# ouguangjun/Leg-KILO

Measured on NVIDIA H100. Metric: LiDAR point-iterations/sec through the ESKF point-to-plane update, higher is better.
Workload: dtype f64

## Files before the change

leg-kilo_b200/csrc/lk_api.cu:

```cuda
#include <cmath>
#include <cstdio>
#include <chrono>
#include <cstring>
#include <mutex>
#include <string>
#include <vector>

#include "lk_host.h"
#include "lk_kernels.h"
#include "lk_mapdev.h"

namespace lk {
int decode_pointcloud2_device(const uint8_t* h_data, uint32_t n, const lk_pc2_layout& L, float blind, int filter_num,
                              double time_scale, float* h_pts_out, float* h_intensity_out, uint32_t* n_out, cudaStream_t s,
                              std::string& err);
int preprocess_scan_device(const float* h_pts_in, uint32_t n, float leaf, float* h_pts_out, uint32_t* n_out,
                           uint32_t* h_bucket_offsets, float* h_bucket_curv, uint32_t* n_buckets, cudaStream_t s,
                           std::string& err);
size_t leg_kinematics_scratch_bytes(uint32_t n);
int leg_kinematics_device(const lk_leg_cfg& cfg, const lk_leg_state* h_in, uint32_t n, int redundancy,
                          lk_leg_track* track, lk_kinimu_meas* h_out, uint32_t* n_out, void* scratch, cudaStream_t s,
                          std::string& err);
}

// ... 22 lines not shown
          Q(clk + align256((size_t)batch * sizeof(lk_stream_clock))),
          chunksL(Q + align256(900 * 8)),
          initsL(chunksL + align256(n_chunksL * sizeof(ChunkDesc))),
          bytes(initsL + align256(n_initsL * sizeof(StepInit))) {}
};

struct OutBlock {
    size_t x = 0, P = 0, clk = 0, n_eff = 0, status = 0, bytes = 0;
    OutBlock() = default;
    explicit OutBlock(int batch)
        : P(align256((size_t)batch * sizeof(lk_state))),
          clk(P + align256((size_t)batch * 900 * 8)),
          n_eff(clk + align256((size_t)batch * sizeof(lk_stream_clock))),
          status(n_eff + align256((size_t)batch * 4)),
          bytes(status + 256) {}
};

}

struct lk_context {
    int device = 0;
    cudaStream_t stream = nullptr;
    std::string err;
    lk_eskf_cfg ec;
    lk_map_cfg mc;
    Globals g;

    MapDevHost map;
    double last_slide_position[3] = {0.0, 0.0, 0.0};

    int batch = 0;
    uint64_t total_pts = 0;
    uint32_t total_chunks = 0, n_steps = 0, max_chunk_pts = 0;
    std::vector<ChunkDesc> h_chunks, h_chunksL;
    InBlock in;
    OutBlock out;
    DevBuf pts, world, sc, step, partial, ticket, fb_list, fb_cnt;
    DevBuf small_in, small_out, fx, fP, fQ, fclk;
    PinnedBuf h_small_in, h_small_out;
    DevView chunks, stepinit, x_in, P_in, clk_in, Q, x, P, clk, n_eff, status;
    DevBuf dbg_ok, dbg_h, dbg_z, dbg_R, dbg_key, tmp, trace, bar;
    DevBuf ins_pts, ins_root, ins_pend, ins_touched, ins_counters, ins_list;
    uint64_t ins_pend_nodes = 0;
    DevBuf mi_pts, mi_small, mi_ipts, mi_root, mi_touched, mi_counters, mi_list;
    PinnedBuf h_mi;
    int trace_on = 0;
    uint32_t trace_seq = 0;
    int lane_cache = 1;
    int use_fused = 1;
    FusedInline inl;
    DevBuf ll;
    uint32_t ll_epoch = 1;
    bool prev_fused = false;
    uint32_t fused_launches = 0, fused_launches_since_check = 0;
    int direct_io = 1, inline_in = 1, coop_launch = 0, pdl = 1, n_sms = 132, slim_p = 1;
    int finishers = 1;
    int fast_insert = 1;
    int fused_insert = 0;
    int debug_records = 0;
    bool direct = false, direct_ran = false, inline_ok = false;
    const float4* direct_pts = nullptr;
    float4* direct_world = nullptr;
    double hprof[8] = {0, 0, 0, 0, 0, 0, 0, 0};
    DevBuf Qc;
    DevBuf leg_scratch;
    std::vector<double> Q_shadow;

    cudaEvent_t ev0 = nullptr, ev1 = nullptr;
    std::vector<cudaEvent_t> kev;
    float last_total_ms = 0, last_residual_ms = 0;
    uint32_t last_launches = 0, last_residual_launches = 0;
    uint32_t acc_launches = 0, acc_residual_launches = 0;
    size_t nev = 0;
    int kernel_timing = 1;
    std::vector<StepInit> h_inits;
    std::vector<uint32_t> h_scan_pts;
    std::vector<uint32_t> h_scan_chunks;
    std::vector<StepInit> h_initsL;
    DevView chunksL, stepinitL;
    uint32_t total_chunksL = 0;

    ~lk_context() {
        for (cudaEvent_t e : kev) cudaEventDestroy(e);
        if (ev0) cudaEventDestroy(ev0);
        if (ev1) cudaEventDestroy(ev1);
        if (stream) cudaStreamDestroy(stream);
    }
};

namespace {

int fail(lk_handle h, int code, const std::string& msg) {
    if (h) h->err = msg;
    else g_create_error = msg;
    return code;
}

struct FusedGate {
    std::mutex m;
    cudaStream_t last = nullptr;
    cudaEvent_t ev = nullptr;
};
FusedGate& fused_gate(int device) {
    static FusedGate gates[64];
    return gates[(device >= 0 && device < 64) ? device : 0];
}

void enter(lk_handle h) {
    cudaSetDevice(h->device);
// ... 181 lines not shown
int lk_init_process_cov(const lk_eskf_cfg* c, double* Q) {
    if (!c || !Q) return LK_ERR_INVALID_ARG;
    for (int i = 0; i < 900; ++i) Q[i] = 0.0;
    const double d[7] = {c->vel_process_cov,     c->acc_bias_process_cov, c->gyr_bias_process_cov, c->imu_acc_process_cov,
                         c->imu_gyr_process_cov, c->kin_bias_process_cov, c->contact_process_cov};
    const int at[7] = {6, 9, 12, 18, 21, 24, 27};
    for (int b = 0; b < 7; ++b)
        for (int k = 0; k < 3; ++k) Q[(at[b] + k) * 30 + at[b] + k] = d[b];
    return LK_OK;
}

int lk_state_default(lk_state* x) {
    if (!x) return LK_ERR_INVALID_ARG;
    std::memset(x, 0, sizeof(*x));
    x->rot[0] = x->rot[4] = x->rot[8] = 1.0;
    x->grav[2] = -9.81;
    return LK_OK;
}

int lk_leg_track_default(lk_leg_track* t) {
    if (!t) return LK_ERR_INVALID_ARG;
    for (int k = 0; k < 4; ++k) t->in_contact[k] = 1;
    t->last_acc_z = 0.0f;
    t->last_gyr_z = 0.0f;
    return LK_OK;
}

int lk_host_alloc(void** p, size_t bytes) {
    if (!p) return LK_ERR_INVALID_ARG;
    cudaError_t e = cudaHostAlloc(p, bytes, cudaHostAllocDefault);
    if (e != cudaSuccess) {
        cudaGetLastError();
        return LK_ERR_OUT_OF_MEMORY;
    }
    return LK_OK;
}

int lk_host_free(void* p) {
    if (p) cudaFreeHost(p);
    return LK_OK;
}

int lk_set_param(lk_handle h, const char* name, double value) {
    if (!h || !name) return LK_ERR_INVALID_ARG;
    using IntKnob = int lk_context::*;
    static const struct {
        const char* name;
        IntKnob knob;
    } knobs[] = {{"kernel_timing", &lk_context::kernel_timing}, {"fused", &lk_context::use_fused},
                 {"lane_cache", &lk_context::lane_cache},       {"fast_insert", &lk_context::fast_insert},
                 {"fused_insert", &lk_context::fused_insert},   {"coop_launch", &lk_context::coop_launch},
                 {"pdl", &lk_context::pdl},                     {"slim_p", &lk_context::slim_p},
                 {"direct_io", &lk_context::direct_io},         {"inline_in", &lk_context::inline_in},
                 {"debug_records", &lk_context::debug_records}, {"finishers", &lk_context::finishers}};
    for (const auto& k : knobs)
        if (!std::strcmp(name, k.name)) {
            h->*k.knob = (int)value;
            return LK_OK;
        }
    if (!std::strcmp(name, "trace")) {
        h->trace_on = (int)value;
        if (h->trace_on) {
            enter(h);
            LK_CUDA(h->err, h->trace.ensure((size_t)(1 << 16) * 8 * 8));
            LK_CUDA(h->err, cudaMemset(h->trace.p, 0, (size_t)(1 << 16) * 8 * 8));
        }
        h->trace_seq = 0;
        return LK_OK;
    }
    return fail(h, LK_ERR_INVALID_ARG, std::string("unknown parameter ") + name);
}

int lk_debug_read(lk_handle h, int what, void* dst, size_t bytes) {
    if (!h || !dst) return LK_ERR_INVALID_ARG;
    if (what == 3) {
        std::memcpy(dst, h->hprof, std::min(bytes, sizeof(h->hprof)));
        std::memset(h->hprof, 0, sizeof(h->hprof));
        return LK_OK;
    }
    enter(h);
    DevBuf* b = what == 0 ? &h->partial : (what == 1 ? &h->sc : &h->trace);
    if (what == 2) h->trace_seq = 0;
    if (bytes > b->cap) bytes = b->cap;
    LK_CUDA(h->err, cudaMemcpy(dst, b->p, bytes, cudaMemcpyDeviceToHost));
    return LK_OK;
}

int lk_sync(lk_handle h) {
    if (!h) return LK_ERR_INVALID_ARG;
    enter(h);
    LK_CUDA(h->err, cudaStreamSynchronize(h->stream));
    return check_stall(h);
}


int lk_map_reserve(lk_handle h, uint64_t max_roots, uint64_t max_nodes, uint64_t max_points) {
    if (!h) return LK_ERR_INVALID_ARG;
    h->map.reserve_roots = max_roots;
    h->map.reserve_nodes = max_nodes;
    h->map.reserve_points = max_points;
    return LK_OK;
}

int lk_map_upload(lk_handle h, const void* blob, size_t bytes) {
    if (!h || !blob) return fail(h, LK_ERR_INVALID_ARG, "null argument");
    enter(h);
    return map_upload_blob(h->map, h->g, blob, bytes, h->stream, h->err);
// ... 158 lines not shown
                    cd.scan = (uint32_t)s;
                    cd.start = q;
                    cd.count = std::min(cs, p1 - q);
                    cd.pad = 0;
                    chunks.push_back(cd);
                }
                in.chunk_end = (uint32_t)chunks.size();
            }
        }
    };
    std::vector<ChunkDesc>& chunks = h->h_chunks;
    std::vector<ChunkDesc>& chunksL = h->h_chunksL;
    std::vector<StepInit>& inits = h->h_inits;
    build_tables(false, chunks, inits);
    bool twoTables = false;
    if (batch >= 2) {
        for (uint32_t b = 0; b < scan_bucket_ptr[batch] && !twoTables; ++b) {
            const uint32_t n = bucket_offsets[b + 1] - bucket_offsets[b];
            twoTables = chunk_size_for(n, true, big_chunk) != chunk_size_for(n, false);
        }
    }
    if (twoTables) build_tables(true, chunksL, h->h_initsL);
    else { chunksL.clear(); h->h_initsL.clear(); }
    h->batch = batch;
    h->h_scan_pts.assign(batch, 0);
    h->h_scan_chunks.assign(batch, 1);
    for (int s2 = 0; s2 < batch; ++s2) {
        h->h_scan_pts[s2] = scan_offsets[s2 + 1] - scan_offsets[s2];
        for (uint32_t k = 0; k < max_buckets; ++k) {
            const StepInit& in = inits[(size_t)k * batch + s2];
            h->h_scan_chunks[s2] = std::max(h->h_scan_chunks[s2], in.chunk_end - in.chunk_begin);
        }
    }
    h->total_pts = total;
    h->total_chunks = (uint32_t)chunks.size();
    h->max_chunk_pts = 0;
    for (const ChunkDesc& cd : chunks) h->max_chunk_pts = std::max(h->max_chunk_pts, cd.count);
    h->n_steps = max_buckets;

    LK_CUDA(h->err, h->pts.ensure(std::max<size_t>(total, 1) * 16));
    LK_CUDA(h->err, h->world.ensure(std::max<size_t>(total, 1) * 16));
    LK_CUDA(h->err, h->sc.ensure((size_t)batch * sizeof(ScanConst)));
    LK_CUDA(h->err, h->step.ensure((size_t)batch * sizeof(ScanStep)));
    LK_CUDA(h->err, h->partial.ensure(2 * std::max<size_t>(std::max(chunks.size(), chunksL.size()), 1) * PARTIAL_STRIDE * 8));
    if (batch >= 2 || h->max_chunk_pts > 256) {
        const size_t nch = std::max<size_t>(std::max(chunks.size(), chunksL.size()), 1);
        LK_CUDA(h->err, h->fb_list.ensure(nch * S2_FB_WARPS * S2_FB_CAP * sizeof(uint16_t)));
        LK_CUDA(h->err, h->fb_cnt.ensure(nch * S2_FB_WARPS * sizeof(uint32_t)));
    }
    if (!h->ll.p) {
        LK_CUDA(h->err, h->ll.ensure(LL_BYTES));
        LK_CUDA(h->err, cudaMemsetAsync(h->ll.p, 0, LL_BYTES, h->stream));
        h->ll_epoch = 1;
    }
    LK_CUDA(h->err, h->ticket.ensure((size_t)batch * 4));
    const InBlock& in = h->in = InBlock(batch, chunks.size(), inits.size(), chunksL.size(), h->h_initsL.size());
    LK_CUDA(h->err, h->small_in.ensure(in.bytes));
    LK_CUDA(h->err, h->h_small_in.ensure(in.bytes));
    char* hs = (char*)h->h_small_in.p;
    if (!chunks.empty()) std::memcpy(hs + in.chunks, chunks.data(), chunks.size() * sizeof(ChunkDesc));
    if (!inits.empty()) std::memcpy(hs + in.inits, inits.data(), inits.size() * sizeof(StepInit));
    std::memcpy(hs + in.x, x, (size_t)batch * sizeof(lk_state));
    std::memcpy(hs + in.P, P, (size_t)batch * 900 * 8);
    std::memcpy(hs + in.clk, clk, (size_t)batch * sizeof(lk_stream_clock));
    std::memcpy(hs + in.Q, Q, 900 * 8);
    if (twoTables) {
        std::memcpy(hs + in.chunksL, chunksL.data(), chunksL.size() * sizeof(ChunkDesc));
        std::memcpy(hs + in.initsL, h->h_initsL.data(), h->h_initsL.size() * sizeof(StepInit));
    }
    char* ds = (char*)h->small_in.p;
    h->chunks.p = ds + in.chunks; h->stepinit.p = ds + in.inits; h->x_in.p = ds + in.x; h->P_in.p = ds + in.P;
    h->clk_in.p = ds + in.clk; h->Q.p = ds + in.Q;
    h->chunksL.p = twoTables ? ds + in.chunksL : ds + in.chunks;
    h->stepinitL.p = twoTables ? ds + in.initsL : ds + in.inits;
    h->total_chunksL = twoTables ? (uint32_t)chunksL.size() : (uint32_t)chunks.size();
    h->out = OutBlock(batch);
    LK_CUDA(h->err, h->small_out.ensure(h->out.bytes));
    LK_CUDA(h->err, h->h_small_out.ensure(h->out.bytes));
    point_outputs(h, (char*)h->small_out.p);
    std::memset((char*)h->h_small_out.p + h->out.status, 0, 4);
    cudaStream_t s = h->stream;
    if (want_direct && h->direct_io && batch == 1 && h->lane_cache && total && h->map.ready() &&
        per_scan_kernel(h, 0, 1, false, false)) {
        const void* dp = pinned_device_ptr(pts);
        void* dw = (dp && world_out) ? pinned_device_ptr(world_out) : nullptr;
        if (dp && (dw || !world_out)) {
            h->direct = true;
            h->direct_pts = (const float4*)dp;
            h->direct_world = dw ? (float4*)dw : h->world.as<float4>();
            point_outputs(h, (char*)h->h_small_out.p);
            if (h->inline_in && max_buckets <= (uint32_t)FUSED_INLINE_STEPS) {
                if (h->Q_shadow.size() != 900 || std::memcmp(h->Q_shadow.data(), Q, 900 * 8) != 0) {
                    LK_CUDA(h->err, h->Qc.ensure(900 * 8));
                    h->Q_shadow.assign(Q, Q + 900);
                    LK_CUDA(h->err, cudaMemcpyAsync(h->Qc.p, h->Q_shadow.data(), 900 * 8, cudaMemcpyHostToDevice, s));
                    LK_CUDA(h->err, cudaStreamSynchronize(s));
                }
                h->inline_ok = true;
                h->Q.p = h->Qc.p;
            }
        }
    }
    if (total && !h->direct) LK_CUDA(h->err, cudaMemcpyAsync(h->pts.p, pts, total * 16, cudaMemcpyHostToDevice, s));
    if (!h->inline_ok) LK_CUDA(h->err, cudaMemcpyAsync(h->small_in.p, h->h_small_in.p, in.bytes, cudaMemcpyHostToDevice, s));
    if (!sync_after) return LK_OK;
    LK_CUDA(h->err, cudaStreamSynchronize(s));
// ... 22 lines not shown
    enter(h);
    LK_CUDA(h->err, cudaEventRecord(h->ev1, h->stream));
    LK_CUDA(h->err, cudaStreamSynchronize(h->stream));
    LK_CUDA(h->err, cudaGetLastError());
    {
        const int rc = check_stall(h);
        if (rc) return rc;
    }
    LK_CUDA(h->err, cudaEventElapsedTime(&h->last_total_ms, h->ev0, h->ev1));
    float rms = 0;
    for (size_t i = 0; i + 1 < h->nev; i += 2) {
        float ms = 0;
        cudaEventElapsedTime(&ms, h->kev[i], h->kev[i + 1]);
        rms += ms;
    }
    h->last_residual_ms = rms;
    h->last_launches = h->acc_launches;
    h->last_residual_launches = h->acc_residual_launches;
    if (total_ms) *total_ms = h->last_total_ms;
    if (residual_kernel_ms) *residual_kernel_ms = rms;
    if (n_kernel_launches) *n_kernel_launches = h->last_launches;
    if (n_residual_launches) *n_residual_launches = h->last_residual_launches;
    return LK_OK;
}

namespace {
struct MeasQueue {
    const lk_imu_meas* d_imu = nullptr;
    const lk_kinimu_meas* d_kin = nullptr;
    const double* stamps = nullptr;
    uint32_t n = 0;
    double gravity = 9.81, acc_norm = 1.0;
};
}

static FusedArgs fused_args(lk_handle h, uint32_t first, int iters, bool insert, const MeasQueue* mq) {
    FusedArgs fa;
    std::memset(&fa, 0, sizeof(fa));
    fa.pts = h->direct ? h->direct_pts : h->pts.as<float4>();
    fa.world = h->direct ? h->direct_world : h->world.as<float4>();
    fa.inits = h->stepinit.as<StepInit>();
    fa.batch = h->batch;
    fa.n_steps = h->n_steps;
    fa.scan = first;
    fa.x_in = h->x_in.as<double>();
    fa.P_in = h->P_in.as<double>();
    fa.clk_in = h->clk_in.as<lk_stream_clock>();
    fa.Q = h->Q.as<double>();
    fa.x = h->x.as<double>();
    fa.P = h->P.as<double>();
    fa.clk = h->clk.as<lk_stream_clock>();
    fa.n_eff = h->n_eff.as<uint32_t>();
    fa.status = h->status.as<uint32_t>();
    fa.ll.chunk_rows = h->ll.as<ulonglong2>();
    fa.ll.group_rows = h->ll.as<ulonglong2>() + (size_t)2 * LL_MAX_CHUNKS * LL_ROW;
    fa.ll.stall = reinterpret_cast<uint32_t*>((char*)h->ll.p + LL_ROWS_BYTES);
    fa.ll.acks = reinterpret_cast<uint32_t*>((char*)h->ll.p + LL_ROWS_BYTES + 64);
    fa.epoch = h->ll_epoch;
    fa.iters = iters;
    fa.lane_cache = h->lane_cache;
    {
        const lk_stream_clock* ck = reinterpret_cast<const lk_stream_clock*>((const char*)h->h_small_in.p + h->in.clk) + first;
        const StepInit& in0 = h->h_inits[first];
        fa.slim_p = h->slim_p && h->n_steps == 1 && !mq && in0.active && in0.t_bucket == ck->last_predict_time &&
                    in0.t_bucket == ck->last_update_time;
    }
    const MapDev md = h->map.dev();
    fa.mv.slots = md.slots;
    fa.mv.hash_mask = md.hash_mask;
    fa.mv.nodes = md.nodes;
    fa.mv.hot = md.hot;
    if (mq) {
        fa.imu = mq->d_imu;
        fa.kin = mq->d_kin;
        fa.n_meas = mq->n;
        fa.gravity = mq->gravity;
        fa.acc_norm = mq->acc_norm;
    }
    {
        const StepInit& in0 = h->h_inits[first];
        const uint32_t sms = (uint32_t)fused_max_blocks(h->device), chunks = h->h_scan_chunks[first];
        if (h->finishers && !insert && fa.n_meas == 0 && h->n_steps == 1 && in0.active && in0.chunk_end - in0.chunk_begin == chunks &&
            chunks > 0 && iters >= 1 && chunks < sms) {
            fa.finishers = std::min(sms - chunks, (uint32_t)LL_MAX_FINISHERS);
            if (h->direct) fa.pts_copy = h->pts.as<float4>();
        }
    }
    fa.ecfg = h->ec;
    fa.trace = h->trace_on ? h->trace.as<unsigned long long>() + (size_t)(h->trace_seq++ % TRACE_AREAS) * TRACE_AREA : nullptr;
    fa.g = h->g;
    if (insert) {
        fa.insert = 1;
        fa.md = md;
        fa.ipts = reinterpret_cast<DevPoint*>(h->ins_pts.p);
        fa.iroot = h->ins_root.as<int>();
        fa.pend = h->ins_pend.as<int>();
        fa.touched = h->ins_touched.as<uint32_t>();
        fa.ins_counters = h->ins_counters.as<uint32_t>() + 2;
    }
    return fa;
}

static int run_fused(lk_handle h, uint32_t first, int iters, bool insert, const MeasQueue* mq, bool timed) {
    cudaStream_t s = h->stream;
    FusedInline* inl = nullptr;
    if (h->inline_ok) {
        const char* hs = (const char*)h->h_small_in.p;
        inl = &h->inl;
        std::memcpy(inl->x, hs + h->in.x, sizeof(inl->x));
        std::memcpy(inl->P, hs + h->in.P, sizeof(inl->P));
        std::memcpy(inl->clk, hs + h->in.clk, sizeof(inl->clk));
        std::memcpy(inl->steps, h->h_inits.data(), h->h_inits.size() * sizeof(StepInit));
    }
    const uint32_t need = h->n_steps * ((uint32_t)iters + 2u) + 1u;
    if (h->ll_epoch > 0xE0000000u || need > 0x10000000u) {
        if (need > 0x10000000u) return fail(h, LK_ERR_INVALID_ARG, "steps x iters too large for one launch");
        LK_CUDA(h->err, cudaMemsetAsync(h->ll.p, 0, LL_BYTES, s));
        h->ll_epoch = 1;
        h->prev_fused = false;
    }
    const FusedArgs fa = fused_args(h, first, iters, insert, mq);
    const uint32_t grid = insert ? (uint32_t)fused_max_blocks(h->device) : h->h_scan_chunks[first] + fa.finishers;
    h->ll_epoch += need;
    if (insert) h->prev_fused = false;
    if (timed) { cudaEventRecord(kev_get(h, h->nev++), s); h->prev_fused = false; }
    const int mode = h->coop_launch ? FUSED_LAUNCH_COOPERATIVE : ((h->pdl && h->prev_fused) ? FUSED_LAUNCH_PDL : FUSED_LAUNCH_PLAIN);
    {
        FusedGate& gate = fused_gate(h->device);
        std::lock_guard<std::mutex> lock(gate.m);
        if (gate.last && gate.last != s) {
            if (!gate.ev) LK_CUDA(h->err, cudaEventCreateWithFlags(&gate.ev, cudaEventDisableTiming));
            LK_CUDA(h->err, cudaEventRecord(gate.ev, gate.last));
            LK_CUDA(h->err, cudaStreamWaitEvent(s, gate.ev, 0));
        }
        gate.last = s;
        LK_CUDA(h->err, launch_scan_fused(fa, inl, grid, s, mode));
    }
    h->prev_fused = true;
    ++h->fused_launches_since_check;
    if (timed) { cudaEventRecord(kev_get(h, h->nev++), s); h->prev_fused = false; }
    ++h->acc_launches;
    ++h->acc_residual_launches;
    h->direct_ran = h->direct;
    return LK_OK;
}

static int run_kernels(lk_handle h, uint32_t first, uint32_t count, int iters, bool update_map, const MeasQueue* mq,
                       bool timed) {
    cudaStream_t s = h->stream;
    const int batch = h->batch;
    const bool big = count >= 2 && !h->h_initsL.empty();
    const std::vector<StepInit>& tin = big ? h->h_initsL : h->h_inits;
    const ChunkDesc* d_chunks = big ? h->chunksL.as<ChunkDesc>() : h->chunks.as<ChunkDesc>();
    const StepInit* d_inits = big ? h->stepinitL.as<StepInit>() : h->stepinit.as<StepInit>();
    uint32_t small_parity = 0;
    uint32_t mi = 0;
    if (mq) {
        LK_CUDA(h->err, cudaMemcpyAsync(h->x.as<lk_state>() + first, h->x_in.as<lk_state>() + first, sizeof(lk_state), cudaMemcpyDeviceToDevice, s));
        LK_CUDA(h->err, cudaMemcpyAsync(h->P.as<double>() + (size_t)first * 900, h->P_in.as<double>() + (size_t)first * 900, 900 * 8, cudaMemcpyDeviceToDevice, s));
        LK_CUDA(h->err, cudaMemcpyAsync(h->clk.as<lk_stream_clock>() + first, h->clk_in.as<lk_stream_clock>() + first, sizeof(lk_stream_clock), cudaMemcpyDeviceToDevice, s));
        LK_CUDA(h->err, cudaMemsetAsync(h->n_eff.as<uint32_t>() + first, 0, 4, s));
    }
    for (uint32_t k = 0; k < h->n_steps; ++k) {
        const StepInit* hin = tin.data() + (size_t)k * batch;
        uint32_t c0 = hin[first].chunk_begin, c1 = hin[first + count - 1].chunk_end;
        uint32_t m_obs0 = mi, m_obs1 = mi;
        if (mq && hin[first].active) {
            while (m_obs1 < mq->n && mq->stamps[m_obs1] < hin[first].t_bucket) ++m_obs1;
            mi = m_obs1;
        }
        const PredictArgs pa = predict_args(h, d_inits + (size_t)k * batch, (k == 0 && !mq) ? 1 : 0, first, count);
        if (mq && count == 1 && hin[first].active)
            launch_obs_predict_prepare(pa, mq->d_imu ? mq->d_imu + m_obs0 : nullptr, mq->d_kin ? mq->d_kin + m_obs0 : nullptr,
                                       m_obs1 - m_obs0, h->ec, mq->gravity, mq->acc_norm, s);
        else
            launch_predict_prepare(pa, s);
        ++h->acc_launches;
        for (int it = 0; it < iters; ++it) {
            ResidualArgs ra = residual_args(h, d_chunks);
            ra.chunk_first = c0;
            ra.last_iter = (it == iters - 1) ? 1 : 0;
            if (timed) cudaEventRecord(kev_get(h, h->nev++), s);
            if (count >= 2 || h->max_chunk_pts > 256) {
                launch_residual_stream2(ra, c1 - c0, s);
                launch_residual_fallback(ra, c1 - c0, s);
                launch_scan_tail(ra, first, count, s);
                if (c1 > c0) h->acc_launches += 2;
            } else {
                launch_residual(ra, c1 - c0, false, !update_map, s);
            }
// ... 489 lines not shown
```

leg-kilo_b200/csrc/lk_fused.cu:

```cuda
#include "lk_insert.cuh"
#include "lk_kernels.h"
#include "lk_obs.cuh"
#include "lk_pass.cuh"
#include "lk_predict.cuh"
#include "lk_solve.cuh"

namespace lk {

namespace {

#define FT(slot) do { if (a.trace && threadIdx.x == 0 && (slot) < 32) a.trace[(size_t)blockIdx.x * 32 + (slot)] = gtime(); } while (0)
#define FTI(slot) do { if (it_global < 3) FT(slot); } while (0)
#define FTS(slot) do { if (a.trace && blockIdx.x == 0 && threadIdx.x == 0 && k < 64) a.trace[(size_t)gridDim.x * 32 + (size_t)k * 8 + (slot)] = gtime(); } while (0)
#ifndef LK_HOP_TRACE
#define LK_HOP_TRACE 0
#endif
#define FT_HOPS() ((LK_HOP_TRACE && a.trace && it_global < 3) \
                       ? a.trace + (size_t)gridDim.x * 32 + 64 * 8 + (size_t)blockIdx.x * 16 + it_global * LL_HOP_SLOTS : nullptr)

constexpr int BLOCK = FB;
constexpr int WARPS = BLOCK / 32;

struct PredictScratch {
    double F[900];
    double T[900];
    double Ps[900];
    ObsScratch obs;
};

template <bool HOT>
struct FusedSmemT {
    BlockFilter f;
    ScanConst sc;
    double slice[WARPS * 32];
    double clk[2];
    union {
        PredictScratch pr;
        PassSmem<BLOCK, HOT> pass;
    } u;
};
typedef FusedSmemT<true> FusedSmem;

struct FusedSmemIns {
    FusedSmemT<false> base;
    WarpTile wt[WARPS];
    MapDev md;
    Globals g;
};

__device__ __noinline__ void fused_insert_phase2(FusedSmemIns* si, const uint32_t* touched, const int* iroot, const DevPoint* ipts,
                                                 int* pend, uint32_t n_touched, uint32_t n_bucket) {
    const int lane = threadIdx.x & 31, warp = threadIdx.x >> 5;
    MapDev md = si->md;
    WarpTile* wt = si->wt + warp;
    for (uint32_t t = blockIdx.x * (uint32_t)WARPS + (uint32_t)warp; t < n_touched; t += gridDim.x * (uint32_t)WARPS)
        warp_insert_root_scan(md, si->g, wt, __ldcg(&touched[t]), iroot, ipts, n_bucket, pend, lane);
}

static_assert(sizeof(PredictScratch) <= sizeof(((PassSmem<BLOCK, true>*)0)->tile) &&
                  sizeof(PredictScratch) <= sizeof(((PassSmem<BLOCK, false>*)0)->tile),
              "predict scratch must not reach the mbarriers");
static_assert(sizeof(FusedSmemIns) <= 227 * 1024, "one block per SM");
static_assert(sizeof(FusedSmem) + 1024 <= 132 * 1024, "the batch-of-one kernel's stack frames must fit in L1");

int carveout_percent(size_t smem, int dev) {
    int per_sm = 0, per_block = 0;
    cudaDeviceGetAttribute(&per_sm, cudaDevAttrMaxSharedMemoryPerMultiprocessor, dev);
    cudaDeviceGetAttribute(&per_block, cudaDevAttrReservedSharedMemoryPerBlock, dev);
    if (per_sm <= 0) return 100;
    const size_t need = smem + (size_t)per_block;
    const int pct = (int)((need * 100 + (size_t)per_sm - 1) / (size_t)per_sm);
    return pct < 100 ? pct : 100;
}

template <class SM>
__device__ __noinline__ void fused_predict(SM* sm, const double* Q, double dtc, double dt) {
    if (dtc != 0.0) {
        build_F(sm->u.pr.F, sm->f.x, dtc);
        cov_predict(sm->f.P, sm->u.pr.F, sm->u.pr.T, sm->u.pr.Ps, Q, dtc);
    }
    if (dt != 0.0) {
        if (threadIdx.x == 0) state_predict(sm->f.x, dt);
    }
    fence_proxy_async();
    __syncthreads();
}

template <class SM>
__device__ __noinline__ void fused_drain_queue(SM* sm, const FusedArgs& a, uint32_t& mi, double t_bucket) {
    bool drained = false;
    while (mi < a.n_meas) {
        const double ts = a.imu ? a.imu[mi].stamp : a.kin[mi].stamp;
        if (!(ts < t_bucket)) break;
        block_predict_to(&sm->f, sm->clk, ts, sm->u.pr.F, sm->u.pr.T, sm->u.pr.Ps, a.Q);
        if (a.imu) block_obs_imu<BLOCK>(&sm->f, &sm->u.pr.obs, a.imu + mi, &a.ecfg, a.gravity, a.acc_norm);
        else block_obs_kinimu<BLOCK>(&sm->f, &sm->u.pr.obs, a.kin + mi, &a.ecfg, a.gravity, a.acc_norm);
        if (threadIdx.x == 0) sm->clk[1] = ts;
        __syncthreads();
        ++mi;
        drained = true;
    }
    if (drained) {
        fence_proxy_async();
        __syncthreads();
    }
}

__device__ __forceinline__ float4 world_out(const double* X, double pix, double piy, double piz, bool updated) {
    float4 o;
    o.x = (float)(X[0] * pix + X[1] * piy + X[2] * piz + X[9]);
    o.y = (float)(X[3] * pix + X[4] * piy + X[5] * piz + X[10]);
    o.z = (float)(X[6] * pix + X[7] * piy + X[8] * piz + X[11]);
    o.w = updated ? 255.0f : 0.0f;
    return o;
}

template <class SM>
__device__ __forceinline__ void store_state(SM* sm, const FusedArgs& a, uint32_t n_eff) {
    const int tid = threadIdx.x;
    if (tid < 36) a.x[(size_t)a.scan * 36 + tid] = sm->f.x[tid];
    if (tid < 2) reinterpret_cast<double*>(a.clk + a.scan)[tid] = sm->clk[tid];
    if (tid == 0) {
        a.n_eff[a.scan] = n_eff;
        *a.status = (*reinterpret_cast<volatile uint32_t*>(a.ll.stall) ? 1u : 0u) | (*reinterpret_cast<volatile uint32_t*>(&lk_stall_note[0]) ? 2u : 0u);
    }
}

template <class SM>
__device__ __noinline__ void fused_finish(SM* sm, const FusedArgs& a, const StepInit& in, uint32_t n_chunks, uint32_t it_global,
                                          bool updated, bool dep_waited) {
    const int tid = threadIdx.x;
    const uint32_t fi = blockIdx.x - n_chunks, nf = gridDim.x - n_chunks;
    if (!dep_waited) asm volatile("griddepcontrol.wait;" ::: "memory");
    ll_sum_chunk_rows<WARPS>(a.ll, it_global & 1u, a.epoch + it_global, n_chunks, sm->u.pr.F, sm->f.acc);
    FTI(3 + it_global * 4);
    const uint32_t n = block_solve_state(&sm->f);
    FTI(4 + it_global * 4);
    if (n > 0) {
        updated = true;
        if (tid == 0) sm->clk[1] = in.t_bucket;
    }
    const float4* pts = a.pts;
    if (a.pts_copy) {
        __threadfence();
        pts = a.pts_copy;
    }
    constexpr int U = 8;
    const uint32_t step = nf * BLOCK;
    for (uint32_t i0 = in.pt_begin + fi * BLOCK + tid; i0 < in.pt_end; i0 += U * step) {
        float4 q[U];
#pragma unroll
        for (int u = 0; u < U; ++u)
            if (i0 + u * step < in.pt_end) q[u] = __ldcg(pts + i0 + u * step);
#pragma unroll
        for (int u = 0; u < U; ++u)
            if (i0 + u * step < in.pt_end) {
                PointCtx p;
                imu_point(q[u], a.g, p);
                a.world[i0 + u * step] = world_out(sm->f.x, p.pix, p.piy, p.piz, updated);
            }
    }
    FT(20);
    if (n > 0) cov_prep(&sm->f, BLOCK);
    __syncthreads();
    for (uint32_t e = fi * BLOCK + tid; e < 900; e += nf * BLOCK)
        a.P[(size_t)a.scan * 900 + e] = n > 0 ? cov_entry(&sm->f, (int)e) : sm->f.P[e];
    FT(21);
    if (fi == 0) store_state(sm, a, n);
    FT(22);
}

template <bool INL> struct InlineSel { typedef FusedInline type; };
template <> struct InlineSel<false> { typedef FusedNoInline type; };

__device__ __forceinline__ void grid_sync(const FusedArgs& a, uint32_t& sync_idx) {
    __threadfence();
    __syncthreads();
    if (threadIdx.x < 32) (void)ll_allreduce(a.ll, sync_idx & 1u, a.epoch + sync_idx, blockIdx.x, gridDim.x, 0.0, (int)threadIdx.x);
    ++sync_idx;
    __syncthreads();
    __threadfence();
    fence_proxy_async_global();
}

template <bool OBS, bool INL, bool INS>
__global__ void __launch_bounds__(BLOCK, 1) k_scan_fused(const __grid_constant__ FusedArgs a,
                                                         const __grid_constant__ typename InlineSel<INL>::type inl) {
    extern __shared__ __align__(16) unsigned char smem_raw[];
    FusedSmemT<!INS>* sm = reinterpret_cast<FusedSmemT<!INS>*>(smem_raw);
    const int tid = threadIdx.x, lane = tid & 31, warp = tid >> 5;
    const uint32_t scan = a.scan;
    const bool finisher = blockIdx.x + a.finishers >= gridDim.x;
    asm volatile("griddepcontrol.launch_dependents;" ::: "memory");
    FT(0);
    {
        const double* Pin;
        const double* xin;
        const double* cin;
        if constexpr (INL) { Pin = inl.P; xin = inl.x; cin = inl.clk; }
        else { Pin = a.P_in + (size_t)scan * 900; xin = a.x_in + (size_t)scan * 36; cin = reinterpret_cast<const double*>(a.clk_in + scan); }
        if (a.slim_p && !finisher && (a.finishers || blockIdx.x != 0)) {
            if (tid < 180) sm->f.P[(tid / 6) * 30 + tid % 6] = Pin[(tid / 6) * 30 + tid % 6];
        } else {
            for (int e = tid; e < 900; e += BLOCK) sm->f.P[e] = Pin[e];
        }
        if (tid < 36) sm->f.x[tid] = xin[tid];
        if (tid < 2) sm->clk[tid] = cin[tid];
    }
    if constexpr (INS) {
        FusedSmemIns* si = reinterpret_cast<FusedSmemIns*>(smem_raw);
        WarpTile* wt = si->wt + warp;
        if (lane == 0) {
            mbar_init(&wt->bar, 1);
            wt->phase = 0;
        }
        if (tid == 0) si->md = a.md;
        if (tid < (int)(sizeof(Globals) / 4)) reinterpret_cast<uint32_t*>(&si->g)[tid] = reinterpret_cast<const uint32_t*>(&a.g)[tid];
    }
    pass_init(&sm->u.pass);
    FT(1);
    uint32_t n_eff_total = 0;
    uint32_t phase = 0;
    uint32_t it_global = 0;
    uint32_t cslot = 0;
    uint32_t mi = 0;
    bool dep_waited = false;

    for (uint32_t k = 0; k < a.n_steps; ++k) {
        StepInit in;
        if constexpr (INL) in = inl.steps[k];
        else in = a.inits[(size_t)k * a.batch + scan];
        if (!in.active) continue;
        const uint32_t n_chunks = in.chunk_end - in.chunk_begin;
        const uint32_t my_start = in.pt_begin + blockIdx.x * (uint32_t)BLOCK;
        const uint32_t my_count = blockIdx.x < n_chunks ? min((uint32_t)BLOCK, in.pt_end - my_start) : 0u;
        float4 pre = make_float4(0.f, 0.f, 0.f, 0.f);
        if ((uint32_t)tid < my_count) pre = __ldg(a.pts + my_start + tid);
        FTS(0);
        if constexpr (OBS) fused_drain_queue(sm, a, mi, in.t_bucket);
        FTS(1);
        const double dtc = in.t_bucket - sm->clk[1];
        const double dt = in.t_bucket - sm->clk[0];
        if (dtc != 0.0 || dt != 0.0) fused_predict(sm, a.Q, dtc, dt);
        if (tid == 0) sm->clk[0] = in.t_bucket;
        FTS(2);
        bool updated = false, cov_pending = false;
        uint32_t n_last = 0;
        LaneCache lc;
        lc.have = 0;
        const bool more_steps = k + 1 < a.n_steps;
        for (int it = 0; it < a.iters; ++it, ++it_global) {
            scan_const_from(&sm->f, &sm->sc);
            __syncthreads();
            double acc[32];
#pragma unroll
            for (int i = 0; i < 32; ++i) acc[i] = 0.0;
            if (!a.lane_cache && lc.have == 2) lc.have = 1;
            points_pass<BLOCK, INS>(&sm->u.pass, phase, my_count, sm->sc, a.mv, a.g, lc, pre,
                                    [&](uint32_t, const Row& row) { accumulate_row(row, acc); });
            FTI(14 + it_global);
            const double tot = warp_transpose_sum(acc, lane);
            sm->slice[warp * 32 + lane] = tot;
            __syncthreads();
            FTI(2 + it_global * 4);
            if (it == 0) FTS(3);
            const bool last = it == a.iters - 1;
            if (!OBS && !INS && a.finishers && last) {
                if (finisher) {
                    fused_finish(sm, a, in, n_chunks, it_global, updated, dep_waited);
                } else {
                    if (!dep_waited) asm volatile("griddepcontrol.wait;" ::: "memory");
                    if (a.pts_copy) {
                        if ((uint32_t)tid < my_count) a.pts_copy[my_start + tid] = pre;
                        __threadfence();
                        __syncthreads();
                    }
                    if (warp == 0) {
                        double v = 0.0;
#pragma unroll
                        for (int w = 0; w < WARPS; ++w) v += sm->slice[w * 32 + lane];
                        ll_publish_row(a.ll, it_global & 1u, a.epoch + it_global, blockIdx.x, v, lane);
                    }
                }
                FT(31);
                return;
            }
            if (warp == 0) {
                double v = 0.0;
#pragma unroll
                for (int w = 0; w < WARPS; ++w) v += sm->slice[w * 32 + lane];
                if (!dep_waited) {
                    FT(23);
                    asm volatile("griddepcontrol.wait;" ::: "memory");
                    FT(24);
                }
                sm->f.acc[lane] = ll_allreduce(a.ll, it_global & 1u, a.epoch + it_global, blockIdx.x, n_chunks, v, lane, FT_HOPS(),
                                               a.finishers, it_global >= 2);
            }
            dep_waited = true;
            __syncthreads();
            FTI(3 + it_global * 4);
            if (it == 0) FTS(4);
            const uint32_t n = block_solve_state(&sm->f);
            FTI(4 + it_global * 4);
            if (n > 0) {
                updated = true;
                if (tid == 0) sm->clk[1] = in.t_bucket;
                if (last) cov_pending = INS || more_steps || blockIdx.x == 0;
            }
            n_last = n;
        }
        n_eff_total += n_last;
        FTS(5);
        if constexpr (!INS) {
            if ((uint32_t)tid < my_count) a.world[my_start + tid] = world_out(sm->f.x, lc.pix, lc.piy, lc.piz, updated);
            FT(20);
            if (cov_pending) block_cov_update<BLOCK>(&sm->f);
        } else {
            if (cov_pending) block_cov_update<BLOCK>(&sm->f);
            __syncthreads();
            scan_const_from(&sm->f, &sm->sc);
            __syncthreads();
            MapDev md = a.md;
            const uint32_t n_bucket = in.pt_end - in.pt_begin;
            if ((uint32_t)tid < my_count) {
                DevPoint p;
                make_insert_point(lc.pix, lc.piy, lc.piz, lc.pbx, lc.pby, lc.pbz, sm->sc, a.g, p);
                const uint32_t li = my_start + tid - in.pt_begin;
                a.ipts[li] = p;
                float4 o;
                o.x = (float)p.pw[0]; o.y = (float)p.pw[1]; o.z = (float)p.pw[2];
                o.w = updated ? 255.0f : 0.0f;
                a.world[my_start + tid] = o;
                a.iroot[li] = insert_register_point(md, a.g, p, a.pend, a.touched, &a.ins_counters[cslot]);
            }
            grid_sync(a, it_global);
            FTS(6);
            {
                const uint32_t n_touched = __ldcg(&a.ins_counters[cslot]);
                if (blockIdx.x == 0 && tid == 0) a.ins_counters[cslot ^ 1u] = 0;
                fused_insert_phase2(reinterpret_cast<FusedSmemIns*>(smem_raw), a.touched, a.iroot, a.ipts, a.pend, n_touched, n_bucket);
                cslot ^= 1u;
            }
            grid_sync(a, it_global);
            FTS(7);
        }
    }
// ... 80 lines not shown
```

leg-kilo_b200/csrc/lk_kernels.h:

```cpp
#pragma once
#include <cuda_runtime.h>

#include "lk_device.cuh"
#include "lk_llsync.cuh"
#include "lk_plane.cuh"

namespace lk {

struct StepInit {
    uint32_t chunk_begin, chunk_end;
    uint32_t pt_begin, pt_end;
    double t_bucket;
    uint32_t active;
    uint32_t pad;
};

struct ResidualArgs {
    const float4* pts;
    const HashSlot* slots;
    uint32_t hash_mask;
    const MapNode* nodes;
    const HotRec* hot;
    const ChunkDesc* chunks;
    uint32_t chunk_first;
// ... 49 lines not shown

struct ReprojectArgs {
    const float4* pts;
    float4* world;
    const ChunkDesc* chunks;
    uint32_t chunk_first;
    const ScanConst* sc;
    const ScanStep* step;
    Globals g;
};
void launch_reproject(const ReprojectArgs& a, uint32_t n_chunks, cudaStream_t s);


void launch_filter_obs(double* x, double* P, const double* Q, lk_stream_clock* clk, const lk_imu_meas* imu,
                       const lk_kinimu_meas* kin, uint32_t n, const lk_eskf_cfg& cfg, double gravity, double acc_norm,
                       cudaStream_t s);
void launch_update_by_points(double* x, double* P, uint32_t n, const double* h, const double* z, const double* r,
                             cudaStream_t s);

constexpr int FUSED_INLINE_STEPS = 64;
struct FusedInline {
    double x[36];
    double P[900];
    double clk[2];
    StepInit steps[FUSED_INLINE_STEPS];
};
struct FusedNoInline {
    int unused;
};

struct FusedArgs {
    const float4* pts;
    float4* world;
    const StepInit* inits;
    int batch;
    uint32_t n_steps;
    uint32_t scan;
    const double* x_in;
    const double* P_in;
    const lk_stream_clock* clk_in;
    const double* Q;
    double* x;
    double* P;
    lk_stream_clock* clk;
    uint32_t* n_eff;
    uint32_t* status;
    LLView ll;
    uint32_t epoch;
    int iters;
    int lane_cache;
    int slim_p;
    uint32_t finishers;
    float4* pts_copy;
    MapView mv;
    const lk_imu_meas* imu;
    const lk_kinimu_meas* kin;
    uint32_t n_meas;
    double gravity, acc_norm;
    lk_eskf_cfg ecfg;
    unsigned long long* trace;
    Globals g;
    int insert;
    MapDev md;
    DevPoint* ipts;
    int* iroot;
    int* pend;
    uint32_t* touched;
    uint32_t* ins_counters;
};
enum { FUSED_LAUNCH_PLAIN = 0, FUSED_LAUNCH_COOPERATIVE = 1, FUSED_LAUNCH_PDL = 2 };
size_t fused_smem_bytes();
int fused_max_blocks(int device);
int fused_read_stall(uint32_t out[8]);
cudaError_t launch_scan_fused(const FusedArgs& a, const FusedInline* inl, uint32_t grid, cudaStream_t s, int mode);

struct PerDeviceOnce {
    bool done[64] = {};
    bool first() {
        int d = 0;
        cudaGetDevice(&d);
        if (d < 0 || d >= 64) return true;
        if (done[d]) return false;
        done[d] = true;
        return true;
    }
};

}
```

leg-kilo_b200/csrc/lk_llsync.cuh:

```cuda
#pragma once
#include <cuda_runtime.h>
#include <stdint.h>

#include "lk_async.cuh"

namespace lk {

constexpr int LK_GROUP = 8;
constexpr int LL_ROW = 32;
constexpr int LL_MAX_CHUNKS = 160;
constexpr int LL_MAX_GROUPS = (LL_MAX_CHUNKS + LK_GROUP - 1) / LK_GROUP;
constexpr int LL_REPLICAS = 4;
constexpr int LL_COPIES = LL_REPLICAS + 1;
constexpr int LL_MAX_FINISHERS = 24;

struct LLView {
    ulonglong2* chunk_rows;
    ulonglong2* group_rows;
    uint32_t* stall;
    uint32_t* acks;
};
constexpr size_t LL_ROWS_BYTES = (size_t)2 * (LL_MAX_CHUNKS + LL_COPIES * LL_MAX_GROUPS) * LL_ROW * sizeof(ulonglong2);
constexpr size_t LL_BYTES = LL_ROWS_BYTES + 64 + 2 * LL_MAX_FINISHERS * sizeof(uint32_t);
constexpr uint32_t LL_SPIN_LIMIT = 1u << 23;
constexpr int LL_HOP_SLOTS = 5;

__device__ __forceinline__ void ll_store(ulonglong2* p, double v, uint32_t tag) {
    const unsigned long long b = (unsigned long long)__double_as_longlong(v);
    const unsigned long long t = (unsigned long long)tag << 32;
    const unsigned long long w0 = (b & 0xffffffffull) | t, w1 = (b >> 32) | t;
    asm volatile("st.relaxed.gpu.global.v2.u64 [%0], {%1, %2};" ::"l"(p), "l"(w0), "l"(w1) : "memory");
}

__device__ __forceinline__ void ll_give_up(uint32_t* stall, uint32_t tag, uint32_t r0, uint32_t n, int lane) {
    if (atomicCAS(stall, 0u, 1u) == 0u) {
        stall[1] = blockIdx.x; stall[2] = tag; stall[3] = r0; stall[4] = n; stall[5] = (uint32_t)lane;
        __threadfence();
    }
}

template <int N, bool KEEP>
__device__ __forceinline__ double ll_sum_rows(const ulonglong2* rows, uint32_t r0, uint32_t n, uint32_t tag, int lane,
                                              uint32_t* stall, uint32_t& rounds, double first = 0.0, bool have_first = false) {
    static_assert(N <= 32, "one bit per row");
    const ulonglong2* p = rows + (size_t)r0 * LL_ROW + lane;
    unsigned long long w0[N], w1[N];
    const unsigned long long want = ((unsigned long long)tag << 32);
    uint32_t spins = 0;
    if constexpr (!KEEP) {
        bool all;
        do {
#pragma unroll
            for (int k = 0; k < N; ++k)
                if ((uint32_t)k < n && !(have_first && k == 0))
                    asm volatile("ld.relaxed.gpu.global.v2.u64 {%0, %1}, [%2];" : "=l"(w0[k]), "=l"(w1[k]) : "l"(p + (size_t)k * LL_ROW));
            all = true;
#pragma unroll
            for (int k = 0; k < N; ++k)
                if ((uint32_t)k < n && !(have_first && k == 0))
                    all = all && ((w0[k] & 0xffffffff00000000ull) == want) && ((w1[k] & 0xffffffff00000000ull) == want);
            ++spins;
            if (!all && ((spins & 0xfffu) == 0u)) {
                if (spins >= LL_SPIN_LIMIT || *reinterpret_cast<volatile uint32_t*>(stall) != 0u) {
                    ll_give_up(stall, tag, r0, n, lane);
                    break;
                }
            }
        } while (!all);
    } else {
        uint32_t todo = (n >= 32u ? 0xffffffffu : (1u << n) - 1u) & (have_first ? ~1u : ~0u);
        while (true) {
#pragma unroll
            for (int k = 0; k < N; ++k)
                if ((todo >> k) & 1u)
                    asm volatile("ld.relaxed.gpu.global.v2.u64 {%0, %1}, [%2];" : "=l"(w0[k]), "=l"(w1[k]) : "l"(p + (size_t)k * LL_ROW));
#pragma unroll
            for (int k = 0; k < N; ++k)
                if (((todo >> k) & 1u) && ((w0[k] & 0xffffffff00000000ull) == want) && ((w1[k] & 0xffffffff00000000ull) == want))
                    todo &= ~(1u << k);
            ++spins;
            if (todo == 0u) break;
            if ((spins & 0xfffu) == 0u) {
                if (spins >= LL_SPIN_LIMIT || *reinterpret_cast<volatile uint32_t*>(stall) != 0u) {
                    ll_give_up(stall, tag, r0, n, lane);
                    break;
                }
            }
        }
    }
    rounds = spins;
    double s = 0.0;
#pragma unroll
    for (int k = 0; k < N; ++k)
        if ((uint32_t)k < n) {
            const double v = (have_first && k == 0) ? first : __longlong_as_double((long long)((w0[k] & 0xffffffffull) | (w1[k] << 32)));
            s += v;
        }
    return s;
}

__device__ __forceinline__ void ll_wait_acks(const uint32_t* acks, uint32_t fin, uint32_t tag, int lane, uint32_t* stall) {
    uint32_t spins = 0;
    bool mine = (uint32_t)lane >= fin;
    while (!__all_sync(0xffffffffu, mine)) {
        if (!mine) {
            uint32_t w;
            asm volatile("ld.acquire.gpu.global.u32 %0, [%1];" : "=r"(w) : "l"(acks + lane) : "memory");
            mine = w == tag;
        }
        if ((++spins & 0xfffu) == 0u && (spins >= LL_SPIN_LIMIT || *reinterpret_cast<volatile uint32_t*>(stall) != 0u)) {
            ll_give_up(stall, tag, 0, fin, lane);
            break;
        }
    }
}

__device__ __forceinline__ double ll_allreduce(const LLView& ll, uint32_t parity, uint32_t tag, uint32_t b, uint32_t n_chunks,
                                               double v, int lane, unsigned long long* hops = nullptr, uint32_t fin = 0,
                                               bool acks_due = false) {
    constexpr size_t COPY = (size_t)LL_MAX_GROUPS * LL_ROW;
    ulonglong2* crows = ll.chunk_rows + (size_t)parity * LL_MAX_CHUNKS * LL_ROW;
    ulonglong2* grows = ll.group_rows + (size_t)parity * LL_COPIES * COPY;
    uint32_t* acks = ll.acks + (size_t)parity * LL_MAX_FINISHERS;
    const uint32_t n_groups = (n_chunks + LK_GROUP - 1) / LK_GROUP;
    uint32_t r1 = 0, r2 = 0;
    if (b < n_chunks) {
        if ((b % LK_GROUP) == 0) {
            if (hops && lane == 0) hops[0] = gtime();
            const uint32_t n = min((uint32_t)LK_GROUP, n_chunks - b);
            const double s = ll_sum_rows<LK_GROUP, false>(crows, b, n, tag, lane, ll.stall, r1, v, true);
            if (hops && lane == 0) hops[1] = gtime();
            ulonglong2* g = grows + (size_t)(b / LK_GROUP) * LL_ROW + lane;
            if (fin && acks_due) ll_wait_acks(acks, fin, tag - 2u, lane, ll.stall);
#pragma unroll
            for (int r = 0; r < LL_REPLICAS; ++r) ll_store(g + (size_t)r * COPY, s, tag);
            if (fin) ll_store(g + (size_t)LL_REPLICAS * COPY, s, tag);
            if (hops && lane == 0) hops[2] = gtime();
        } else {
            ll_store(crows + (size_t)b * LL_ROW + lane, v, tag);
            if (hops && lane == 0) hops[0] = gtime();
        }
    }
    const bool finisher = fin && b >= n_chunks;
    const double t = ll_sum_rows<LL_MAX_GROUPS, true>(grows + (size_t)(finisher ? LL_REPLICAS : b % LL_REPLICAS) * COPY, 0, n_groups,
                                                      tag, lane, ll.stall, r2);
    if (finisher) {
        __syncwarp();
        if (lane == 0) asm volatile("st.release.gpu.global.u32 [%0], %1;" ::"l"(acks + (b - n_chunks)), "r"(tag) : "memory");
    }
    if (hops) {
        r1 = __reduce_max_sync(0xffffffffu, r1);
        r2 = __reduce_max_sync(0xffffffffu, r2);
        if (lane == 0) {
            hops[3] = gtime();
            hops[4] = (unsigned long long)r1 | ((unsigned long long)r2 << 32);
        }
    }
    return t;
}

__device__ __forceinline__ void ll_publish_row(const LLView& ll, uint32_t parity, uint32_t tag, uint32_t b, double v, int lane) {
    ll_store(ll.chunk_rows + ((size_t)parity * LL_MAX_CHUNKS + b) * LL_ROW + lane, v, tag);
}

template <int NWARPS>
__device__ __forceinline__ void ll_sum_chunk_rows(const LLView& ll, uint32_t parity, uint32_t tag, uint32_t n_chunks, double* gs,
                                                  double* out) {
    const int tid = threadIdx.x, lane = tid & 31, warp = tid >> 5;
    const ulonglong2* crows = ll.chunk_rows + (size_t)parity * LL_MAX_CHUNKS * LL_ROW;
    const uint32_t n_groups = (n_chunks + LK_GROUP - 1) / LK_GROUP;
    for (uint32_t g = (uint32_t)warp; g < n_groups; g += NWARPS) {
        uint32_t rounds;
        gs[g * 32 + lane] = ll_sum_rows<LK_GROUP, false>(crows, g * LK_GROUP, min((uint32_t)LK_GROUP, n_chunks - g * LK_GROUP), tag,
                                                         lane, ll.stall, rounds);
    }
    __syncthreads();
    if (tid < 32) {
        double t = 0.0;
        for (uint32_t g = 0; g < n_groups; ++g) t += gs[g * 32 + tid];
        out[tid] = t;
    }
    __syncthreads();
}

}
```

Baseline: 3.146 billion.

## Replace PDL griddepcontrol.wait with fine-grained release acks from previous launch finishers

Double-buffers the low-latency allreduce row/ack buffers across consecutive fused launches, and has finisher blocks publish release acks once they have consumed the chunk rows. With PDL active, chunk blocks of the next launch skip griddepcontrol.wait before the allreduce and instead check or spin on the previous launch's finisher acks. This lets the next scan's allreduce start before the prior grid fully completes. It adds spin-wait logic and extra memory-ordering subtleties that could risk correctness or stalls.

```diff
diff --git a/leg-kilo_b200/csrc/lk_api.cu b/leg-kilo_b200/csrc/lk_api.cu
--- a/leg-kilo_b200/csrc/lk_api.cu
+++ b/leg-kilo_b200/csrc/lk_api.cu
@@ -98,9 +98,12 @@
     DevBuf ll;
     uint32_t ll_epoch = 1;
     bool prev_fused = false;
+    uint32_t ll_set = 0;
+    struct { uint32_t tag, parity, fin; } ll_last[2] = {};
     uint32_t fused_launches = 0, fused_launches_since_check = 0;
     int direct_io = 1, inline_in = 1, coop_launch = 0, pdl = 1, n_sms = 132, slim_p = 1;
     int finishers = 1;
+    int late_dep_wait = 1;
     int fast_insert = 1;
     int fused_insert = 0;
     int debug_records = 0;
@@ -388,7 +391,8 @@
                  {"fused_insert", &lk_context::fused_insert},   {"coop_launch", &lk_context::coop_launch},
                  {"pdl", &lk_context::pdl},                     {"slim_p", &lk_context::slim_p},
                  {"direct_io", &lk_context::direct_io},         {"inline_in", &lk_context::inline_in},
-                 {"debug_records", &lk_context::debug_records}, {"finishers", &lk_context::finishers}};
+                 {"debug_records", &lk_context::debug_records}, {"finishers", &lk_context::finishers},
+                 {"late_dep_wait", &lk_context::late_dep_wait}};
     for (const auto& k : knobs)
         if (!std::strcmp(name, k.name)) {
             h->*k.knob = (int)value;
@@ -653,6 +657,8 @@
         LK_CUDA(h->err, h->ll.ensure(LL_BYTES));
         LK_CUDA(h->err, cudaMemsetAsync(h->ll.p, 0, LL_BYTES, h->stream));
         h->ll_epoch = 1;
+        h->ll_set = 0;
+        for (auto& l : h->ll_last) l = {0, 0, 0};
     }
     LK_CUDA(h->err, h->ticket.ensure((size_t)batch * 4));
     const InBlock& in = h->in = InBlock(batch, chunks.size(), inits.size(), chunksL.size(), h->h_initsL.size());
@@ -781,10 +787,10 @@
     fa.clk = h->clk.as<lk_stream_clock>();
     fa.n_eff = h->n_eff.as<uint32_t>();
     fa.status = h->status.as<uint32_t>();
-    fa.ll.chunk_rows = h->ll.as<ulonglong2>();
-    fa.ll.group_rows = h->ll.as<ulonglong2>() + (size_t)2 * LL_MAX_CHUNKS * LL_ROW;
+    fa.ll.chunk_rows = h->ll.as<ulonglong2>() + (size_t)h->ll_set * LL_SET_ROWS;
+    fa.ll.group_rows = fa.ll.chunk_rows + LL_CHUNK_ROWS;
     fa.ll.stall = reinterpret_cast<uint32_t*>((char*)h->ll.p + LL_ROWS_BYTES);
-    fa.ll.acks = reinterpret_cast<uint32_t*>((char*)h->ll.p + LL_ROWS_BYTES + 64);
+    fa.ll.acks = reinterpret_cast<uint32_t*>((char*)h->ll.p + LL_ROWS_BYTES + 64) + (size_t)h->ll_set * LL_SET_ACKS;
     fa.epoch = h->ll_epoch;
     fa.iters = iters;
     fa.lane_cache = h->lane_cache;
@@ -847,13 +853,22 @@
         LK_CUDA(h->err, cudaMemsetAsync(h->ll.p, 0, LL_BYTES, s));
         h->ll_epoch = 1;
         h->prev_fused = false;
-    }
-    const FusedArgs fa = fused_args(h, first, iters, insert, mq);
+        h->ll_set = 0;
+        for (auto& l : h->ll_last) l = {0, 0, 0};
+    }
+    FusedArgs fa = fused_args(h, first, iters, insert, mq);
     const uint32_t grid = insert ? (uint32_t)fused_max_blocks(h->device) : h->h_scan_chunks[first] + fa.finishers;
     h->ll_epoch += need;
     if (insert) h->prev_fused = false;
     if (timed) { cudaEventRecord(kev_get(h, h->nev++), s); h->prev_fused = false; }
     const int mode = h->coop_launch ? FUSED_LAUNCH_COOPERATIVE : ((h->pdl && h->prev_fused) ? FUSED_LAUNCH_PDL : FUSED_LAUNCH_PLAIN);
+    auto& last = h->ll_last[h->ll_set];
+    if (h->late_dep_wait && mode == FUSED_LAUNCH_PDL && fa.finishers && last.fin) {
+        fa.late_wait = 1;
+        fa.rel_tag = last.tag;
+        fa.rel_fin = last.fin;
+        fa.rel_acks = fa.ll.acks + (size_t)last.parity * LL_MAX_FINISHERS;
+    }
     {
         FusedGate& gate = fused_gate(h->device);
         std::lock_guard<std::mutex> lock(gate.m);
@@ -865,6 +880,10 @@
         gate.last = s;
         LK_CUDA(h->err, launch_scan_fused(fa, inl, grid, s, mode));
     }
+    last.fin = fa.finishers;
+    last.tag = fa.epoch + (uint32_t)iters - 1u;
+    last.parity = ((uint32_t)iters - 1u) & 1u;
+    h->ll_set ^= 1u;
     h->prev_fused = true;
     ++h->fused_launches_since_check;
     if (timed) { cudaEventRecord(kev_get(h, h->nev++), s); h->prev_fused = false; }
diff --git a/leg-kilo_b200/csrc/lk_fused.cu b/leg-kilo_b200/csrc/lk_fused.cu
--- a/leg-kilo_b200/csrc/lk_fused.cu
+++ b/leg-kilo_b200/csrc/lk_fused.cu
@@ -34,6 +34,7 @@
     ScanConst sc;
     double slice[WARPS * 32];
     double clk[2];
+    uint32_t rel_ok;
     union {
         PredictScratch pr;
         PassSmem<BLOCK, HOT> pass;
@@ -132,7 +133,7 @@
     const int tid = threadIdx.x;
     const uint32_t fi = blockIdx.x - n_chunks, nf = gridDim.x - n_chunks;
     if (!dep_waited) asm volatile("griddepcontrol.wait;" ::: "memory");
-    ll_sum_chunk_rows<WARPS>(a.ll, it_global & 1u, a.epoch + it_global, n_chunks, sm->u.pr.F, sm->f.acc);
+    ll_sum_chunk_rows<WARPS>(a.ll, it_global & 1u, a.epoch + it_global, n_chunks, fi, sm->u.pr.F, sm->f.acc);
     FTI(3 + it_global * 4);
     const uint32_t n = block_solve_state(&sm->f);
     FTI(4 + it_global * 4);
@@ -206,6 +207,12 @@
         }
         if (tid < 36) sm->f.x[tid] = xin[tid];
         if (tid < 2) sm->clk[tid] = cin[tid];
+    }
+    if (a.late_wait && warp == WARPS - 1) {
+        uint32_t w = 0;
+        if ((uint32_t)lane < a.rel_fin) asm volatile("ld.acquire.gpu.global.u32 %0, [%1];" : "=r"(w) : "l"(a.rel_acks + lane) : "memory");
+        const bool ok = __all_sync(0xffffffffu, (uint32_t)lane >= a.rel_fin || w >= a.rel_tag);
+        if (lane == 0) sm->rel_ok = ok;
     }
     if constexpr (INS) {
         FusedSmemIns* si = reinterpret_cast<FusedSmemIns*>(smem_raw);
@@ -267,9 +274,13 @@
             const bool last = it == a.iters - 1;
             if (!OBS && !INS && a.finishers && last) {
                 if (finisher) {
-                    fused_finish(sm, a, in, n_chunks, it_global, updated, dep_waited);
+                    fused_finish(sm, a, in, n_chunks, it_global, updated, dep_waited && !a.late_wait);
                 } else {
-                    if (!dep_waited) asm volatile("griddepcontrol.wait;" ::: "memory");
+                    if (!dep_waited || a.late_wait) {
+                        FT(23);
+                        asm volatile("griddepcontrol.wait;" ::: "memory");
+                        FT(24);
+                    }
                     if (a.pts_copy) {
                         if ((uint32_t)tid < my_count) a.pts_copy[my_start + tid] = pre;
                         __threadfence();
@@ -290,9 +301,15 @@
 #pragma unroll
                 for (int w = 0; w < WARPS; ++w) v += sm->slice[w * 32 + lane];
                 if (!dep_waited) {
-                    FT(23);
-                    asm volatile("griddepcontrol.wait;" ::: "memory");
-                    FT(24);
+                    if (!a.late_wait) {
+                        FT(23);
+                        asm volatile("griddepcontrol.wait;" ::: "memory");
+                        FT(24);
+                    } else {
+                        FT(25);
+                        if (!sm->rel_ok) ll_wait_release(a.rel_acks, a.rel_fin, a.rel_tag, lane, a.ll.stall);
+                        FT(26);
+                    }
                 }
                 sm->f.acc[lane] = ll_allreduce(a.ll, it_global & 1u, a.epoch + it_global, blockIdx.x, n_chunks, v, lane, FT_HOPS(),
                                                a.finishers, it_global >= 2);
diff --git a/leg-kilo_b200/csrc/lk_kernels.h b/leg-kilo_b200/csrc/lk_kernels.h
--- a/leg-kilo_b200/csrc/lk_kernels.h
+++ b/leg-kilo_b200/csrc/lk_kernels.h
@@ -125,6 +125,9 @@
     int slim_p;
     uint32_t finishers;
     float4* pts_copy;
+    uint32_t late_wait;
+    uint32_t rel_tag, rel_fin;
+    const uint32_t* rel_acks;
     MapView mv;
     const lk_imu_meas* imu;
     const lk_kinimu_meas* kin;
diff --git a/leg-kilo_b200/csrc/lk_llsync.cuh b/leg-kilo_b200/csrc/lk_llsync.cuh
--- a/leg-kilo_b200/csrc/lk_llsync.cuh
+++ b/leg-kilo_b200/csrc/lk_llsync.cuh
@@ -20,8 +20,11 @@
     uint32_t* stall;
     uint32_t* acks;
 };
-constexpr size_t LL_ROWS_BYTES = (size_t)2 * (LL_MAX_CHUNKS + LL_COPIES * LL_MAX_GROUPS) * LL_ROW * sizeof(ulonglong2);
-constexpr size_t LL_BYTES = LL_ROWS_BYTES + 64 + 2 * LL_MAX_FINISHERS * sizeof(uint32_t);
+constexpr size_t LL_CHUNK_ROWS = (size_t)2 * LL_MAX_CHUNKS * LL_ROW;
+constexpr size_t LL_SET_ROWS = LL_CHUNK_ROWS + (size_t)2 * LL_COPIES * LL_MAX_GROUPS * LL_ROW;
+constexpr size_t LL_ROWS_BYTES = 2 * LL_SET_ROWS * sizeof(ulonglong2);
+constexpr size_t LL_SET_ACKS = (size_t)2 * LL_MAX_FINISHERS;
+constexpr size_t LL_BYTES = LL_ROWS_BYTES + 64 + 2 * LL_SET_ACKS * sizeof(uint32_t);
 constexpr uint32_t LL_SPIN_LIMIT = 1u << 23;
 constexpr int LL_HOP_SLOTS = 5;
 
@@ -107,6 +110,22 @@
             uint32_t w;
             asm volatile("ld.acquire.gpu.global.u32 %0, [%1];" : "=r"(w) : "l"(acks + lane) : "memory");
             mine = w == tag;
+        }
+        if ((++spins & 0xfffu) == 0u && (spins >= LL_SPIN_LIMIT || *reinterpret_cast<volatile uint32_t*>(stall) != 0u)) {
+            ll_give_up(stall, tag, 0, fin, lane);
+            break;
+        }
+    }
+}
+
+__device__ __forceinline__ void ll_wait_release(const uint32_t* acks, uint32_t fin, uint32_t tag, int lane, uint32_t* stall) {
+    uint32_t spins = 0;
+    bool mine = (uint32_t)lane >= fin;
+    while (!__all_sync(0xffffffffu, mine)) {
+        if (!mine) {
+            uint32_t w;
+            asm volatile("ld.acquire.gpu.global.u32 %0, [%1];" : "=r"(w) : "l"(acks + lane) : "memory");
+            mine = w >= tag;
         }
         if ((++spins & 0xfffu) == 0u && (spins >= LL_SPIN_LIMIT || *reinterpret_cast<volatile uint32_t*>(stall) != 0u)) {
             ll_give_up(stall, tag, 0, fin, lane);
@@ -164,8 +183,8 @@
 }
 
 template <int NWARPS>
-__device__ __forceinline__ void ll_sum_chunk_rows(const LLView& ll, uint32_t parity, uint32_t tag, uint32_t n_chunks, double* gs,
-                                                  double* out) {
+__device__ __forceinline__ void ll_sum_chunk_rows(const LLView& ll, uint32_t parity, uint32_t tag, uint32_t n_chunks, uint32_t fi,
+                                                  double* gs, double* out) {
     const int tid = threadIdx.x, lane = tid & 31, warp = tid >> 5;
     const ulonglong2* crows = ll.chunk_rows + (size_t)parity * LL_MAX_CHUNKS * LL_ROW;
     const uint32_t n_groups = (n_chunks + LK_GROUP - 1) / LK_GROUP;
@@ -175,6 +194,7 @@
                                                          lane, ll.stall, rounds);
     }
     __syncthreads();
+    if (tid == 0) asm volatile("st.release.gpu.global.u32 [%0], %1;" ::"l"(ll.acks + (size_t)parity * LL_MAX_FINISHERS + fi), "r"(tag) : "memory");
     if (tid < 32) {
         double t = 0.0;
         for (uint32_t g = 0; g < n_groups; ++g) t += gs[g * 32 + tid];
```

Result: faster. 3.245 billion, median of 6 (+3.1%).
